# andrewli77/combinatorial-rl-tasks

Measured on NVIDIA B200. Metric: env_steps_per_sec, higher is better.
Workload: dtype f32

## Files before the change

combinatorial_rl_tasks_b200/_lib.py:

```python
import ctypes
import os

HERE = os.path.dirname(os.path.abspath(__file__))
LIB_PATH = os.environ.get('CRL_B200_LIB') or os.path.join(HERE, 'libcrl_b200.so')

c_void_p, c_int32, c_int64, c_uint32, c_uint64, c_double = (
    ctypes.c_void_p, ctypes.c_int32, ctypes.c_int64, ctypes.c_uint32, ctypes.c_uint64, ctypes.c_double)

TASK_TSP, TASK_TTSP, TASK_CM = 0, 1, 2
SEED_INCREMENT, SEED_FIXED_RANGE = 0, 1
STEP_AUTO_RESET, STEP_PHYSICS_ONLY, STEP_CHAINED, STEP_CHAIN_START, STEP_TRACK_ROWS = 1, 2, 4, 8, 16
STEP_GOALS, STEP_WAIT, STEP_ACTION_COUNTER, STEP_NO_ZONE_OBS, STEP_HOST_PLANES = 32, 64, 128, 512, 1024
STEP_ZONE_OBS_DELTA = 2048
ABI_VERSION = 9
NUM_PLANES = 23

SYMBOLS = ['crl_abi_version', 'crl_strerror', 'crl_plane_bytes', 'crl_step_bytes', 'crl_reset',
           'crl_prefetch_layouts', 'crl_prefetch_publish', 'crl_reset_from_layout', 'crl_step', 'crl_step_host',
           'crl_host_call_create', 'crl_host_call_step', 'crl_host_call_destroy',
           'crl_set_goal', 'crl_goal_query', 'crl_set_qpos_qvel',
           'crl_get_qpos_qvel', 'crl_gae', 'crl_check_state', 'crl_counters_read',
           'crl_encoder_packed_bytes', 'crl_encoder_pack', 'crl_zone_encode', 'crl_zone_encode_state',
           'crl_encoder_head_packed_bytes', 'crl_encoder_pack_head', 'crl_encoder_head',
           'crl_encoder_workspace_bytes', 'crl_encoder_forward',
           'crl_encoder_precise_packed_bytes', 'crl_encoder_pack_precise', 'crl_zone_encode_precise',
           'crl_encoder_backward_workspace_bytes', 'crl_zone_encode_backward',
           'crl_frame_capture', 'crl_zone_encode_frames', 'crl_zone_encode_backward_frames', 'crl_frames_zone_obs']
FRAME_NO_LAYOUT = 0xffffffff


class CrlConfig(ctypes.Structure):
    _fields_ = [('task', c_int32), ('num_envs', c_int32), ('num_zones', c_int32), ('num_steps', c_int32),
                ('frameskip', c_int32), ('max_cooldown', c_int32), ('seed_mode', c_int32),
# ... 36 lines not shown
            '(nvcc, sm_100a).  This package has no CPU fallback.')
    lib = ctypes.CDLL(LIB_PATH)
    P = ctypes.POINTER
    lib.crl_abi_version.restype = ctypes.c_int
    lib.crl_strerror.restype = ctypes.c_char_p
    lib.crl_strerror.argtypes = [ctypes.c_int]
    lib.crl_plane_bytes.argtypes = [P(CrlConfig), P(c_int64), c_int32]
    lib.crl_step_bytes.argtypes = [P(CrlConfig), P(c_int64), P(c_int64)]
    lib.crl_reset.argtypes = [P(CrlConfig), P(CrlState), P(CrlOut), c_void_p, c_void_p]
    lib.crl_prefetch_layouts.argtypes = [P(CrlConfig), P(CrlState), c_int32, c_uint32, c_void_p]
    lib.crl_prefetch_publish.argtypes = [P(CrlState), c_uint32, c_void_p]
    lib.crl_reset_from_layout.argtypes = [P(CrlConfig), P(CrlState), P(CrlOut), P(CrlLayoutIn), c_void_p,
                                          c_int32, c_void_p]
    lib.crl_step.argtypes = [P(CrlConfig), P(CrlState), c_void_p, P(CrlOut), c_uint32, c_uint64, c_uint64,
                             c_void_p]
    lib.crl_step_host.argtypes = [P(CrlConfig), P(CrlState), c_void_p, c_void_p, P(CrlOut), P(CrlOut),
                                  c_uint32, c_void_p]
    lib.crl_host_call_create.argtypes = [P(CrlConfig), P(CrlState), P(CrlOut), P(CrlOut), c_uint32, P(c_void_p)]
    lib.crl_host_call_step.argtypes = [c_void_p, c_void_p, c_void_p]
    lib.crl_host_call_destroy.argtypes = [c_void_p]
    lib.crl_host_call_destroy.restype = None
    lib.crl_set_goal.argtypes = [P(CrlConfig), P(CrlState), c_void_p, c_void_p]
    lib.crl_goal_query.argtypes = [P(CrlConfig), P(CrlState), c_void_p, c_void_p, c_void_p, c_void_p]
    lib.crl_set_qpos_qvel.argtypes = [P(CrlConfig), P(CrlState), c_void_p, c_void_p, c_void_p, c_int32,
                                      c_void_p]
    lib.crl_get_qpos_qvel.argtypes = [P(CrlConfig), P(CrlState), c_void_p, c_void_p, c_void_p, c_int32,
                                      c_void_p]
    lib.crl_gae.argtypes = [c_void_p, c_void_p, c_void_p, c_void_p, c_double, c_double, c_int32, c_int32,
                            c_void_p, c_void_p, c_void_p]
    lib.crl_check_state.argtypes = [P(CrlConfig), P(CrlState), c_void_p, c_void_p]
# ... 35 lines not shown
```

combinatorial_rl_tasks_b200/csrc/crl_core.cuh:

```cuda
#pragma once
#include <math.h>
#include <stdint.h>

#if defined(__CUDACC__)
#define CRL_HD __host__ __device__ __forceinline__
#define CRL_HD_COLD inline __host__ __device__ __noinline__
#else
#define CRL_HD inline
#define CRL_HD_COLD inline
#endif

namespace crl {

constexpr double kPi = 3.14159265358979323846;
constexpr double kH = 0.002;
constexpr double kMSphere = 4.0 / 3.0 * kPi * 0.1 * 0.1 * 0.1;
constexpr double kMBox = 8.0 * 0.05 * 0.05 * 0.05;
constexpr double kMass = kMSphere + kMBox;
constexpr double kCom = kMBox * 0.1 / kMass;
constexpr double kIHinge = 0.4 * kMSphere * 0.01 + kMBox / 3.0 * (0.0025 + 0.0025) + kMBox * 0.01;
constexpr double kDampLin = 0.01;
constexpr double kDampYaw = 0.005;
constexpr double kGear = 0.3;
constexpr double kForceLimit = 0.05;
// ... 207 lines not shown
#if defined(__CUDA_ARCH__)
  const double d2 = __dadd_rn(__dmul_rn(dx, dx), __dmul_rn(dy, dy));
#else
  volatile double xx = dx * dx;
  volatile double yy = dy * dy;
  const double d2 = xx + yy;
#endif
  return d2 <= thresh2;
}

CRL_HD bool near_zone(float X, float Y, float zx, float zy, float r2_guard) {
  const float dx = zx - X, dy = zy - Y;
  return dx * dx + dy * dy <= r2_guard;
}

CRL_HD int popcount32(uint32_t x) {
#if defined(__CUDA_ARCH__)
  return __popc(x);
#else
  return __builtin_popcount(x);
#endif
}

CRL_HD int hamming(uint32_t colours, int n) {
  const uint32_t field = n >= 16 ? 0x55555555u : ((1u << (2 * n)) - 1u) & 0x55555555u;
  const uint32_t lo = colours & field, hi = (colours >> 1) & field;
  const int ng = popcount32(lo & ~hi), nr = popcount32(hi & ~lo);
  const int nb = popcount32(field & ~(lo | hi));
  const int to_b = 2 * ng + nr, to_g = 2 * nr + nb, to_r = 2 * nb + ng;
  int m = to_b < to_g ? to_b : to_g;
// ... 44 lines not shown
```

combinatorial_rl_tasks_b200/csrc/crl_kernels.cu:

```cuda
#include <cuda_runtime.h>

#include <atomic>
#include <stdint.h>
#include <stdio.h>
#include <string.h>

#include "../../include/crl_b200.h"
#include "crl_core.cuh"

namespace crl {

#ifndef CRL_THREADS
#define CRL_THREADS 64
#endif
constexpr int kThreads = CRL_THREADS;
constexpr unsigned kFull = 0xffffffffu;

struct KParams {
  int B, num_steps, frameskip, max_cd, seed_mode, env_offset;
  long long min_seed, max_seed;
  double thresh2;
  float r2_guard;
  double bonus_per_step;
  double beta_a, beta_b;
// ... 23 lines not shown
  float* zone_obs_host;
  unsigned long long* result_dev;
  int32_t* goal;
  const float2* bank_zone_xy;
  const float4* bank_origin;
  const uint32_t* bank_task;
  const float4* fixed;
  uint32_t init_hi;
  uint32_t walled;
  const float2* actions;
  float4* obs;
  float* zone_obs;
  unsigned long long* result;
  float* shaped;
  const uint8_t* mask;
};

constexpr uint32_t kParBit = 0x8000u, kHiMask = 0x7fffu;

template <int TASK>
struct ZoneDim { static constexpr int Z = (TASK == CRL_TASK_TSP) ? 6 : 7; };

#ifndef CRL_REGS_N15
#define CRL_REGS_N15 112
#endif
template <int N>
struct MaxRegs { static constexpr int v = N > 8 ? CRL_REGS_N15 : 80; };

template <int N>
struct Env {
// ... 157 lines not shown

constexpr uint32_t kSlotEmpty = 0u, kSlotLayoutDone = 2u, kSlotClaimed = 3u, kSlotReady = 16u;

__device__ __forceinline__ uint32_t ld_acquire_u32(const uint32_t* p) {
  uint32_t v;
  asm volatile("ld.acquire.gpu.global.u32 %0, [%1];" : "=r"(v) : "l"(p) : "memory");
  return v;
}
__device__ __forceinline__ uint32_t ld_relaxed_u32(const uint32_t* p) {
  uint32_t v;
  asm volatile("ld.relaxed.gpu.global.u32 %0, [%1];" : "=r"(v) : "l"(p) : "memory");
  return v;
}
__device__ __forceinline__ void st_release_u32(uint32_t* p, uint32_t v) {
  asm volatile("st.release.gpu.global.u32 [%0], %1;" :: "l"(p), "r"(v) : "memory");
}

template <int TASK, int N>
__device__ __forceinline__ bool reset_from_slot(const KParams& p, int e, Env<N>& env) {
  const int B = p.B;
  const uint32_t par = env.hi >> 15;
  uint32_t episode, col_word = 0u;
  long long chosen;
  float4 o;
  uint32_t* slot_flag = nullptr;
  if (p.bank_zone_xy) {
    episode = p.episode[e];
    chosen = choose_seed(p, e, episode);
    if (chosen < p.min_seed || chosen > p.max_seed) return false;
    const size_t k = (size_t)(chosen - p.min_seed);
// ... 496 lines not shown
    row[0] = row0;
    row[1] = row1;
  }
  asm volatile("fence.proxy.async.shared::cta;" ::: "memory");
  __syncwarp();
  const int n_valid = max(0, min(32, B - warp_env0));
  if (lane == 0 && n_valid > 0) {
    const uint32_t saddr = (uint32_t)__cvta_generic_to_shared(stage);
    float4* gdst = obs + 2 * (size_t)warp_env0;
    asm volatile("cp.async.bulk.global.shared::cta.bulk_group [%0], [%1], %2;"
                 :: "l"(gdst), "r"(saddr), "r"((uint32_t)n_valid * 32u) : "memory");
    asm volatile("cp.async.bulk.commit_group;" ::: "memory");
  }
}

template <int TASK, int N>
__device__ __forceinline__ void load_env(const KParams& p, int e, Env<N>& env) {
  const float4 ps = p.pose[e];
  const float4 ax = p.aux[e];
#pragma unroll
  for (int i = 0; i < N; ++i) env.zone[i] = p.zone_xy[(size_t)i * p.B + e];
  if (TASK == CRL_TASK_TTSP) {
#pragma unroll
    for (int j = 0; j < (N + 1) / 2; ++j) env.tmax[j] = p.zone_tmax[(size_t)j * p.B + e];
  }
  if (TASK == CRL_TASK_CM) env.cd = p.cooldown[e];
  env.b.X = ps.x; env.b.Y = ps.y; env.b.phi = ps.z; env.b.vx = ps.w;
  env.b.vy = ax.x; env.b.w = ax.y; env.ep_return = ax.z;
  const uint32_t bits = (uint32_t)__float_as_int(ax.w);
  env.steps = (int)(bits & 0xffffu);
  env.hi = bits >> 16;
}

__device__ __forceinline__ double dist_np(float X, float Y, float zx, float zy) {
  const double dx = (double)zx - (double)X, dy = (double)zy - (double)Y;
  return __dsqrt_rn(__dadd_rn(__dmul_rn(dx, dx), __dmul_rn(dy, dy)));
// ... 13 lines not shown
      __nanosleep(64);
      if (++polls > (1u << 22)) { atomicAdd(p.counters + 7, 1.0); break; }
    }
  }
  __syncwarp();
}

__device__ __forceinline__ void chain_release(const KParams& p, int w, int lane, uint32_t ticket) {
  __syncwarp();
  if (lane == 0) {
    asm volatile("cp.async.bulk.wait_group 0;" ::: "memory");
    if (w < (p.B + 31) / 32) st_release_u32(p.stamp + (p.B + 31) / 32 + w, ticket + 1u);
  }
}

template <int TASK, int N, bool EXT, bool FIXED = false>
__global__ void __maxnreg__(MaxRegs<N>::v) step_kernel(const __grid_constant__ KParams p) {
  constexpr int ROW = N * ZoneDim<TASK>::Z;
  extern __shared__ __align__(128) float smem[];
  const int lane = threadIdx.x & 31, warp = threadIdx.x >> 5;
  const int e = blockIdx.x * kThreads + threadIdx.x;
  const int warp_env0 = blockIdx.x * kThreads + warp * 32;
  const bool valid = e < p.B;
  float* stage = smem + warp * (32 * ROW);
  uint32_t ticket = 0u;
  const bool ticketed = (p.flags & (CRL_STEP_CHAINED | CRL_STEP_CHAIN_START)) != 0u;
  if (ticketed) {
    ticket = chain_ticket(p, warp_env0 >> 5, lane);
    asm volatile("griddepcontrol.launch_dependents;" :: "r"(ticket) : "memory");
  } else {
    asm volatile("griddepcontrol.launch_dependents;" ::: "memory");
  }
  if (p.flags & CRL_STEP_CHAINED) {
    chain_wait(p, warp_env0 >> 5, lane, ticket);
  } else {
    asm volatile("griddepcontrol.wait;" ::: "memory");
  }

  uint32_t act_base = 0u;
  uint32_t* act_cnt = nullptr;
  if (!p.actions && (p.flags & CRL_STEP_ACTION_COUNTER) && lane == 0 && warp_env0 < p.B) {
    act_cnt = p.act_count + (warp_env0 >> 5);
    act_base = ld_relaxed_u32(act_cnt);
  }
  Env<N> env;
  float2 act = make_float2(0.f, 0.f);
  if (valid) load_env<TASK, N>(p, e, env);
  if (!p.actions && (p.flags & CRL_STEP_ACTION_COUNTER)) {
    if (act_cnt) *act_cnt = act_base + 1u;
    act_base = __shfl_sync(kFull, act_base, 0);
  }
  if (valid) {
    if (p.actions) {
      act = p.actions[e];
    } else {
      const unsigned ge = (unsigned)(p.env_offset + e);
      const unsigned long long si = p.step_index + act_base;
      U4 ctr{ge, (uint32_t)si, (uint32_t)(si >> 32), kTagAction};
      const U4 r = philox4x32(ctr, (uint32_t)p.action_seed, (uint32_t)(p.action_seed >> 32));
      act = make_float2(2.f * u01(r.x) - 1.f, 2.f * u01(r.y) - 1.f);
    }
  } else {
    env.b = Body{0.f, 0.f, 0.f, 0.f, 0.f, 0.f};
    env.ep_return = 0.f; env.steps = 0; env.hi = 0u; env.cd = make_uint2(0u, 0u);
#pragma unroll
    for (int i = 0; i < N; ++i) env.zone[i] = make_float2(1e9f, 1e9f);
#pragma unroll
    for (int j = 0; j < (N + 1) / 2; ++j) env.tmax[j] = 0xffffffffu;
  }

  const bool parked = EXT && (p.flags & CRL_STEP_WAIT) && valid && env.steps == kParkedSteps;
  const bool live = valid && !parked;
  const bool revive = EXT && parked && (p.flags & CRL_STEP_AUTO_RESET);
  const bool goals = EXT && (p.flags & CRL_STEP_GOALS);
  int goal_zone = -1;
  float gzx = 0.f, gzy = 0.f;
  double dist_before = 0.0;
  Body old_b = env.b;
  bool reached = false, park_now = false;
  if (goals && live) {
    goal_zone = p.goal[e];
// ... 3 lines not shown
      dist_before = dist_np(env.b.X, env.b.Y, gzx, gzy);
    }
  }
  int fired_out = -1;
  __shared__ unsigned s_rows_mask[kThreads / 32];
  const bool some_rows = p.zone_obs_host || (p.flags & CRL_STEP_ZONE_OBS_DELTA);
  if (some_rows && lane == 0) s_rows_mask[warp] = 0u;
  bool fresh = false;
  if (!(p.flags & CRL_STEP_PHYSICS_ONLY)) {
    bool row_changed = TASK == CRL_TASK_TTSP && !(p.flags & CRL_STEP_HOST_PLANES);
    if (TASK == CRL_TASK_CM) {
      row_changed = (env.cd.x | env.cd.y) != 0u;
      env.cd.x = cd_dec4(env.cd.x); env.cd.y = cd_dec4(env.cd.y);
    }
    uint32_t cand = 0u;
#pragma unroll
    for (int i = 0; i < N; ++i)
      if (near_zone(env.b.X, env.b.Y, env.zone[i].x, env.zone[i].y, p.r2_guard)) cand |= 1u << i;
    if (TASK == CRL_TASK_CM) {
      if (cand) {
#pragma unroll
        for (int i = 0; i < N; ++i) if (cd_get(env.cd, i) != 0u) cand &= ~(1u << i);
      }
    } else {
      cand &= ~env.hi;
    }
    int fired = -1;
    while (cand) {
      const int i = __ffs(cand) - 1;
      cand &= cand - 1u;
      float zx = 0.f, zy = 0.f;
#pragma unroll
      for (int j = 0; j < N; ++j) if (j == i) { zx = env.zone[j].x; zy = env.zone[j].y; }
      if (inside_zone(env.b.X, env.b.Y, zx, zy, p.thresh2)) { fired = i; break; }
    }
    int event = 0;
    if (fired >= 0) {
      if (TASK == CRL_TASK_CM) {
        const int old_dist = hamming(env.hi, N);
        const uint32_t col = (env.hi >> (2 * fired)) & 3u;
        const uint32_t nxt = col == 2u ? 0u : col + 1u;
        env.hi = (env.hi & ~(3u << (2 * fired))) | (nxt << (2 * fired));
        cd_set(env.cd, fired, (uint32_t)p.max_cd);
        event = old_dist - hamming(env.hi, N);
      } else {
        env.hi |= 1u << fired;
        event = 1;
      }
// ... 83 lines not shown
        if (left) {
          Env<N> next = env;
          warp_reset<TASK, N, FIXED>(p, left, lane, e, reinterpret_cast<float2*>(stage), par_in, next);
          env = next;
        }
      }
    }
  }
  float c, s;
  if (!EXT) {
    unsigned rows = 0u;
    if (some_rows) {
      __syncwarp();
      rows = s_rows_mask[warp];
    }
    if (!(p.flags & CRL_STEP_NO_ZONE_OBS) && zone_obs_step<TASK, N>(p, env, stage, lane, warp_env0, rows) && !p.zone_obs_host)
      rows = 0u;
    if (rows || p.zone_obs_host) {
      __syncwarp();
      send_rows<TASK, N>(p, p.zone_obs_host ? p.zone_obs_host : p.zone_obs, stage, rows, lane, warp_env0);
    }
    if (fresh) {
      sincosf(env.b.phi, &s, &c);
    } else {
      substeps(env.b, act.x, act.y, p.frameskip, c, s);
      env.b.phi = wrap_pi(env.b.phi);
    }
    if (p.zone_obs_host) {
      store_state_obs_host<TASK, N>(p, env, valid, e, c, s, stage, lane, warp_env0);
    } else if (valid) {
      store_state_obs<TASK, N>(p, env, e, c, s);
    }
  } else {
    if (!(p.flags & CRL_STEP_NO_ZONE_OBS))
      zone_obs_send<TASK, N>(p, env, live || revive, stage, lane, warp_env0, parked && !revive);
    if (p.zone_obs_host) send_rows<TASK, N>(p, p.zone_obs_host, stage, s_rows_mask[warp], lane, warp_env0);
    Body pb = fresh ? old_b : env.b;
    if (p.walled) substeps<CRL_CONTACT_MODEL, true>(pb, act.x, act.y, p.frameskip, c, s, p.extent);
    else substeps(pb, act.x, act.y, p.frameskip, c, s);
    if (fresh) {
      sincosf(env.b.phi, &s, &c);
    } else {
      env.b = pb;
      env.b.phi = wrap_pi(env.b.phi);
    }
    if (goals && live) {
      double shaped = 0.0;
      if (goal_zone >= 0 && !reached) {
// ... 3 lines not shown
      p.shaped[e] = (float)shaped;
    }
    if (parked && goals) p.shaped[e] = 0.f;
    if (parked && !revive) {
      p.obs[2 * (size_t)e] = make_float4(0.f, 0.f, 0.f, 0.f);
      p.obs[2 * (size_t)e + 1] = make_float4(0.f, 0.f, 0.f, 0.f);
    } else if (valid) {
      store_state_obs<TASK, N>(p, env, e, c, s, park_now);
    }
  }
  if (ticketed) {
    chain_release(p, warp_env0 >> 5, lane, ticket);
  } else {
    zone_obs_wait(lane);
  }
}

template <int TASK, int N>
__global__ void __launch_bounds__(kThreads) reset_kernel(const __grid_constant__ KParams p) {
  constexpr int ROW = N * ZoneDim<TASK>::Z;
  extern __shared__ __align__(128) float smem[];
  const int lane = threadIdx.x & 31, warp = threadIdx.x >> 5;
  const int e = blockIdx.x * kThreads + threadIdx.x;
  const int warp_env0 = blockIdx.x * kThreads + warp * 32;
  const bool valid = e < p.B;
  float* stage = smem + warp * (32 * ROW);
  Env<N> env;
  if (valid) load_env<TASK, N>(p, e, env);
  const bool want = valid && (p.mask == nullptr || p.mask[e] != 0);
  const unsigned m = __ballot_sync(kFull, want);
// ... 291 lines not shown

static int fill_params(const CrlConfig* c, const CrlState* st, const CrlOut* out, KParams& p) {
  int rc = check_config(c);
  if (rc) return rc;
  if (!st || !st->pose || !st->aux || !st->zone_xy || !st->seed || !st->episode || !st->origin || !st->counters)
    return CRL_ERR_NULL;
  if (c->task == CRL_TASK_TTSP && !st->zone_tmax) return CRL_ERR_NULL;
  if (c->task == CRL_TASK_CM && !st->cooldown) return CRL_ERR_NULL;
  if (!aligned16(st->pose) || !aligned16(st->aux) || !aligned16(st->zone_xy) || !aligned16(st->origin))
    return CRL_ERR_ALIGN;
  memset(&p, 0, sizeof(p));
  p.B = c->num_envs; p.num_steps = c->num_steps; p.frameskip = c->frameskip; p.max_cd = c->max_cooldown;
  p.seed_mode = c->seed_mode; p.env_offset = c->env_offset; p.min_seed = c->min_seed; p.max_seed = c->max_seed;
  p.thresh2 = sqrt_threshold(c->zone_size);
  p.r2_guard = (float)(c->zone_size * c->zone_size * 1.001 + 1e-5);
  p.bonus_per_step = c->time_saved_reward;
  p.beta_a = c->beta_a; p.beta_b = c->beta_b;
  p.div_steps = cached_div_const(c->num_steps, -65535, 65535);
  p.div_cd = cached_div_const(c->max_cooldown > 0 ? c->max_cooldown : 1, 0, 255);
  if (!p.div_steps.exact || !p.div_cd.exact) return CRL_ERR_CONFIG;
  p.robot_keepout = (float)c->robot_keepout; p.zone_keepout = (float)c->zone_keepout; p.extent = (float)c->extent;
  p.pose = reinterpret_cast<float4*>(st->pose); p.aux = reinterpret_cast<float4*>(st->aux);
  p.zone_xy = reinterpret_cast<float2*>(st->zone_xy); p.zone_tmax = st->zone_tmax;
  p.cooldown = reinterpret_cast<uint2*>(st->cooldown);
  p.seed = reinterpret_cast<long long*>(st->seed); p.episode = st->episode;
  p.origin = reinterpret_cast<float4*>(st->origin); p.counters = st->counters;
  if (st->next_ready) {
    if (!st->next_zone_xy || !st->next_origin || !st->next_seed || (c->task != CRL_TASK_TSP && !st->next_task))
      return CRL_ERR_NULL;
    if (!aligned16(st->next_origin) || !aligned16(st->next_zone_xy)) return CRL_ERR_ALIGN;
// ... 32 lines not shown
}

static int launch_status() { return cudaGetLastError() == cudaSuccess ? CRL_OK : CRL_ERR_LAUNCH; }

#define CRL_DISPATCH(task, n, CALL)                                              \
  do {                                                                           \
    if ((task) == CRL_TASK_TSP && (n) == 15) { CALL(CRL_TASK_TSP, 15); }         \
    else if ((task) == CRL_TASK_TSP && (n) == 5) { CALL(CRL_TASK_TSP, 5); }      \
    else if ((task) == CRL_TASK_TTSP && (n) == 15) { CALL(CRL_TASK_TTSP, 15); }  \
    else if ((task) == CRL_TASK_TTSP && (n) == 5) { CALL(CRL_TASK_TTSP, 5); }    \
    else if ((task) == CRL_TASK_CM && (n) == 6) { CALL(CRL_TASK_CM, 6); }        \
    else return CRL_ERR_UNSUPPORTED;                                             \
  } while (0)

template <int T, int NN>
static void (*pick_step_kernel(bool ext, bool fixed))(const KParams) {
  if (fixed) {
    if constexpr (T == CRL_TASK_TSP && NN == 15) return ext ? step_kernel<T, NN, true, true> : step_kernel<T, NN, false, true>;
    else return nullptr;
  }
  return ext ? step_kernel<T, NN, true> : step_kernel<T, NN, false>;
}

static int set_smem(void (*kernel)(const KParams), size_t bytes) {
  static void (*done_for[32])(const KParams) = {nullptr};
  if (bytes <= 48 * 1024) return CRL_OK;
  for (int i = 0; i < 32; ++i) {
    if (done_for[i] == kernel) return CRL_OK;
    if (done_for[i] == nullptr) {
      if (cudaFuncSetAttribute(kernel, cudaFuncAttributeMaxDynamicSharedMemorySize, (int)bytes) != cudaSuccess)
        return CRL_ERR_DEVICE;
// ... 34 lines not shown
  const int64_t B = c->num_envs, N = c->num_zones, Z = zone_dim(c->task);
  o[0] = 16 * B; o[1] = 16 * B; o[2] = 8 * N * B;
  o[3] = c->task == CRL_TASK_TTSP ? 4 * ((N + 1) / 2) * B : 0;
  o[4] = c->task == CRL_TASK_CM ? 8 * B : 0;
  o[5] = 8 * B; o[6] = 4 * B; o[7] = 16 * B; o[8] = 8 * 8;
  o[9] = 2 * 8 * N * B;
  o[10] = 2 * (c->task == CRL_TASK_TTSP ? 4 * ((N + 1) / 2) * B : (c->task == CRL_TASK_CM ? 4 * B : 0));
  o[11] = 2 * 16 * B; o[12] = 2 * 8 * B; o[13] = 2 * 4 * B;
  o[14] = 32 * B; o[15] = 4 * N * Z * B; o[16] = 8 * B;
  o[17] = 3 * 4 * ((B + 31) / 32);
  o[18] = 16 * (1 + 2 * B);
  o[19] = 16;
  o[20] = 4 * B;
  o[21] = 4 * B;
  o[22] = 16;
  for (int i = 0; i < n && i < CRL_NUM_PLANES; ++i) out_bytes[i] = o[i];
  return CRL_OK;
}

int crl_step_bytes(const CrlConfig* c, int64_t* rd, int64_t* wr) {
  int rc = check_config(c);
  if (rc) return rc;
  if (!rd || !wr) return CRL_ERR_NULL;
  const int64_t N = c->num_zones, Z = zone_dim(c->task);
  int64_t r = 8  + 32  + 8 * N, w = 32 + 8  + 32  + 4 * N * Z;
  if (c->task == CRL_TASK_TTSP) r += 4 * ((N + 1) / 2);
  if (c->task == CRL_TASK_CM) { r += 8; w += 8; }
  *rd = r; *wr = w;
  return CRL_OK;
}

static int step_launch(const CrlConfig* c, const CrlState* st, const float* actions, const CrlOut* out,
                       uint32_t flags, uint64_t action_seed, uint64_t step_index, float* zone_obs_host, void* stream,
                       CrlResult* result_dev = nullptr) {
  KParams p;
  if (!out) return CRL_ERR_NULL;
  int rc = fill_params(c, st, out, p);
  if (rc) return rc;
  p.zone_obs_host = zone_obs_host;
  p.result_dev = reinterpret_cast<unsigned long long*>(result_dev);
  if (result_dev && (!zone_obs_host || !p.row_list)) return CRL_ERR_CONFIG;
  if (actions && (reinterpret_cast<uintptr_t>(actions) & 7u)) return CRL_ERR_ALIGN;
  p.actions = reinterpret_cast<const float2*>(actions);
  p.flags = flags; p.action_seed = action_seed; p.step_index = step_index;
  const bool ticketed = (flags & (CRL_STEP_CHAINED | CRL_STEP_CHAIN_START)) != 0u;
  if (ticketed && !p.stamp) return CRL_ERR_NULL;
  if ((flags & CRL_STEP_TRACK_ROWS) && !p.row_list) return CRL_ERR_NULL;
  if ((flags & CRL_STEP_GOALS) && (!p.goal || !p.shaped)) return CRL_ERR_NULL;
  if ((flags & CRL_STEP_ACTION_COUNTER) && !p.act_count) return CRL_ERR_NULL;
  if (!(flags & CRL_STEP_NO_ZONE_OBS) && !p.zone_obs) return CRL_ERR_NULL;
  if ((flags & CRL_STEP_NO_ZONE_OBS) && (zone_obs_host || (flags & CRL_STEP_TRACK_ROWS))) return CRL_ERR_CONFIG;
  if ((flags & CRL_STEP_HOST_PLANES) && (!zone_obs_host || c->task != CRL_TASK_TTSP)) return CRL_ERR_CONFIG;
  const bool ext = (flags & (CRL_STEP_GOALS | CRL_STEP_WAIT)) != 0u || c->walled != 0u;
  if ((flags & CRL_STEP_ZONE_OBS_DELTA) && (ext || zone_obs_host || (flags & CRL_STEP_NO_ZONE_OBS))) return CRL_ERR_CONFIG;
  if (c->task == CRL_TASK_TTSP) p.flags &= ~CRL_STEP_ZONE_OBS_DELTA;
  static std::atomic<void*> last_chained_stream{reinterpret_cast<void*>(-1)};
  const bool after_chained = last_chained_stream.load(std::memory_order_relaxed) == stream;
  const bool programmatic = (flags & CRL_STEP_CHAINED) || !after_chained;
  last_chained_stream.store((flags & CRL_STEP_CHAINED) ? stream : reinterpret_cast<void*>(-1), std::memory_order_relaxed);
  const int blocks = (p.B + kThreads - 1) / kThreads;
  cudaStream_t s = static_cast<cudaStream_t>(stream);
#define CRL_CALL_STEP(T, NN)                                                        \
  {                                                                                 \
    const size_t sm = (size_t)kThreads * NN * ZoneDim<T>::Z * 4;                    \
    void (*kern)(const KParams) = pick_step_kernel<T, NN>(ext, p.fixed != nullptr); \
    if (!kern) return CRL_ERR_UNSUPPORTED;                                          \
    rc = set_smem(kern, sm);                                                        \
    if (rc) return rc;                                                              \
    cudaLaunchConfig_t lc = {};                                                     \
    lc.gridDim = dim3(blocks); lc.blockDim = dim3(kThreads);                        \
    lc.dynamicSmemBytes = sm; lc.stream = s;                                        \
    cudaLaunchAttribute at[1];                                                      \
    at[0].id = cudaLaunchAttributeProgrammaticStreamSerialization;                  \
    at[0].val.programmaticStreamSerializationAllowed = 1;                           \
    lc.attrs = at; lc.numAttrs = programmatic ? 1 : 0;                              \
    if (cudaLaunchKernelEx(&lc, kern, p) != cudaSuccess) {                          \
      (void)cudaGetLastError();                                                     \
      return CRL_ERR_LAUNCH;                                                        \
    }                                                                               \
  }
  CRL_DISPATCH(c->task, c->num_zones, CRL_CALL_STEP);
  return launch_status();
}

int crl_step(const CrlConfig* c, const CrlState* st, const float* actions, const CrlOut* out,
             uint32_t flags, uint64_t action_seed, uint64_t step_index, void* stream) {
  return step_launch(c, st, actions, out, flags, action_seed, step_index, nullptr, stream);
}

int crl_reset(const CrlConfig* c, const CrlState* st, const CrlOut* out, const uint8_t* mask, void* stream) {
  KParams p;
  if (!out || !out->zone_obs) return CRL_ERR_NULL;
  int rc = fill_params(c, st, out, p);
  if (rc) return rc;
  p.mask = mask;
  const int blocks = (p.B + kThreads - 1) / kThreads;
  cudaStream_t s = static_cast<cudaStream_t>(stream);
#define CRL_CALL_RESET(T, NN)                                                       \
  {                                                                                 \
    const size_t sm = (size_t)kThreads * NN * ZoneDim<T>::Z * 4;                    \
    rc = set_smem(reset_kernel<T, NN>, sm);                                         \
    if (rc) return rc;                                                              \
// ... 259 lines not shown
```

combinatorial_rl_tasks_b200/vec_env.py:

```python
import contextlib
import ctypes

import numpy as np
import torch

from . import _lib
from .config import ENV_SPECS
from .spaces import Box, Dict


_NO_GUARD = contextlib.nullcontext()


class _EnvView:

    def __init__(self, vec, index):
        self._vec, self.index = vec, index
        self.observation_space = vec.observation_space
        self.action_space = vec.action_space

    @property
    def unwrapped(self):
        return self

# ... 39 lines not shown
        self._write_zone_obs = True
        N, Z = spec.num_zones, spec.zone_dim
        self.cfg = _lib.CrlConfig(
            task=spec.task, num_envs=B, num_zones=N, num_steps=spec.num_steps, frameskip=spec.frameskip,
            max_cooldown=spec.max_cooldown,
            seed_mode=_lib.SEED_FIXED_RANGE if seed_mode == 'fixed_range' else _lib.SEED_INCREMENT,
            env_offset=env_offset, min_seed=min_seed, max_seed=max_seed, zone_size=spec.zone_size,
            time_saved_reward=spec.time_saved_reward, beta_a=spec.beta_a, beta_b=spec.beta_b,
            robot_keepout=spec.robot_keepout, zone_keepout=spec.zone_keepout, extent=spec.extent,
            initial_visited=spec.initial_visited, walled=1 if spec.walled else 0)
        dev = self.device
        z = lambda *shape, dtype=torch.float32: torch.zeros(*shape, dtype=dtype, device=dev)
        self.pose = z(B, 4)
        self.aux = z(B, 4)
        self.zone_xy = z(N, B, 2)
        self.zone_tmax = z((N + 1) // 2, B, dtype=torch.int32) if spec.task == _lib.TASK_TTSP else None
        self.cooldown = z(B, 2, dtype=torch.int32) if spec.task == _lib.TASK_CM else None
        self.seeds = z(B, dtype=torch.int64)
        self.episode = z(B, dtype=torch.int32)
        self.origin = z(B, 4)
        self.counters_dev = z(8, dtype=torch.float64)
        self.next_zone_xy = z(2, N, B, 2)
        if spec.task == _lib.TASK_TTSP:
            self.next_task = z(2, (N + 1) // 2, B, dtype=torch.int32)
        elif spec.task == _lib.TASK_CM:
            self.next_task = z(2, B, dtype=torch.int32)
        else:
            self.next_task = None
        self.next_origin = z(2, B, 4)
        self.next_seed = z(2, B, dtype=torch.int64)
# ... 96 lines not shown
         self.need_next_goal, self.out) = binding
        self._mirror_ok = False
        self._zone_obs_ok = False
        self._chain_ok = False

    @property
    def write_zone_obs(self):
        return self._write_zone_obs

    @write_zone_obs.setter
    def write_zone_obs(self, on):
        self._write_zone_obs = bool(on)
        self._mirror_ok = False
        self._zone_obs_ok = False

    def _guard(self):
        return _NO_GUARD if torch.cuda.current_device() == self._dev_index else torch.cuda.device(self.device)

    def _stream(self):
        return ctypes.c_void_p(_raw_stream(self._dev_index))

    def _obs_dict(self):
        return {'zone_obs': self.zone_obs, 'obs': self.obs}

    def _info(self):
        info = {'goal_met': self.goal_met, 'cost': self._cost, 'event': self.event}
        if self.spec.goals:
            info['shaped_reward'] = self.shaped_reward
            info['need_next_goal'] = self.need_next_goal
        return info
# ... 74 lines not shown
                n = xy0.shape[0]
                rot0 = self._as_dev(layout['rot0'], torch.float64).reshape(n)
                zxy = self._as_dev(layout['zone_xy'], torch.float64).reshape(n, self.spec.num_zones, 2)
                tm = self._as_dev(layout['zone_max_steps'], torch.int32) if 'zone_max_steps' in layout else None
                col = self._as_dev(layout['colours'], torch.int32) if 'colours' in layout else None
                ids = None if env_ids is None else self._as_dev(env_ids, torch.int32)
                lay = _lib.CrlLayoutIn(xy0=xy0.data_ptr(), rot0=rot0.data_ptr(), zone_xy=zxy.data_ptr(),
                                       zone_max_steps=None if tm is None else tm.data_ptr(),
                                       colours=None if col is None else col.data_ptr())
                _lib.check(self.lib.crl_reset_from_layout(self.cfg, self.state, self.out, lay,
                                                          None if ids is None else ids.data_ptr(), n,
                                                          self._stream()))
            self.gpu_launches += 1
            self._chain_ok = False
            self._mirror_ok = False
            self._zone_obs_ok = layout is None and mask is None
            if self.prefetch_every and not torch.cuda.is_current_stream_capturing():
                self.prefetch(torch.cuda.current_stream(self.device))
        return self._obs_dict()

    def _step(self, actions, flags, action_seed=0, chained=False):
        if chained:
            flags |= _lib.STEP_CHAINED if self._chain_ok else _lib.STEP_CHAIN_START
        if not flags & _lib.STEP_PHYSICS_ONLY:
            flags |= self._mode_flags
        if not self._write_zone_obs:
            flags |= _lib.STEP_NO_ZONE_OBS
        elif self._zone_obs_ok and not flags & (_lib.STEP_GOALS | _lib.STEP_WAIT) and not self.spec.walled:
            flags |= _lib.STEP_ZONE_OBS_DELTA
        with self._guard():
            if actions is None:
                aptr = None
            else:
                if not (isinstance(actions, torch.Tensor) and actions.is_cuda and actions.dtype == torch.float32
                        and actions.is_contiguous()):
                    actions = self._as_dev(actions, torch.float32)
                assert actions.shape == (self.num_envs, 2)
                aptr = actions.data_ptr()
            si = 0 if flags & _lib.STEP_ACTION_COUNTER else self._step_index
            _lib.check(self.lib.crl_step(self.cfg, self.state, aptr, self.out, flags, action_seed, si, self._stream()))
        self._step_index += 1
        self.gpu_launches += 1
        self._chain_ok = bool(chained)
        self._mirror_ok = False
        self._zone_obs_ok = self._write_zone_obs
        if self.prefetch_every and not torch.cuda.is_current_stream_capturing():
            self.tick()
        return self._obs_dict(), self.reward, self.done, self._info()

    def step(self, actions):
        return self._step(actions, (_lib.STEP_AUTO_RESET if self.auto_reset else 0) | (_lib.STEP_WAIT if self.wait else 0))

    def step_no_reset(self, actions):
        return self._step(actions, _lib.STEP_WAIT if self.wait else 0)

# ... 49 lines not shown
            pin = self._pinned.get(id(actions))
            if pin is not None:
                aptr = pin[1]
            else:
                aptr = h['actions_ptr']
                if actions is not h['np']['actions']:
                    np.copyto(h['np']['actions'], np.asarray(actions, dtype=np.float32).reshape(self.num_envs, 2))
            if torch.cuda.current_device() == self._dev_index:
                rc = self._host_call_step(call, aptr, _raw_stream(self._dev_index))
            else:
                with torch.cuda.device(self.device):
                    rc = self._host_call_step(call, aptr, _raw_stream(self._dev_index))
            if rc:
                _lib.check(rc)
            self.delta_rows = -1
            self._step_index += 1
            self.gpu_launches += 1
            self._chain_ok = False
            self._zone_obs_ok = True
            if self.prefetch_every:
                self.tick()
            return h['ret']
        hn = h['np']
        aptr = h['actions_ptr']
        if actions is not hn['actions']:
            pin = self._pinned.get(id(actions))
            if pin is not None:
                aptr = pin[1]
            else:
                np.copyto(hn['actions'], np.asarray(actions, dtype=np.float32).reshape(self.num_envs, 2))
# ... 5 lines not shown
                src = h['actions'] if aptr == h['actions_ptr'] else self._pinned[id(actions)][0]
                self._actions_dev.copy_(src, non_blocking=True)
                _lib.check(self.lib.crl_step(self.cfg, self.state, self._actions_dev.data_ptr(), self.out, flags, 0,
                                             self._step_index, self._stream()))
                h['zone_obs'].copy_(self.zone_obs.permute(2, 0, 1), non_blocking=True)
                h['obs'].copy_(self.obs, non_blocking=True)
                h['result'].copy_(self.result, non_blocking=True)
                if self.spec.goals:
                    h['shaped'].copy_(self.shaped_reward, non_blocking=True)
                torch.cuda.current_stream(self.device).synchronize()
            else:
                _lib.check(self.lib.crl_step_host(self.cfg, self.state, aptr,
                                                  self._actions_dev.data_ptr(), self.out, h['out'],
                                                  flags, self._stream()))
        self.delta_rows = self.num_envs
        self._step_index += 1
        self.gpu_launches += 1
        self._chain_ok = False
        self._mirror_ok = True
        self._zone_obs_ok = True
        if self.prefetch_every:
            self.tick()
        return h['ret']

    def _host_call(self, auto_reset, wait):
        h = self._host
        flags = (_lib.STEP_AUTO_RESET if auto_reset else 0) | (_lib.STEP_WAIT if wait else 0) | self._mode_flags
        if self.spec.task == _lib.TASK_TTSP:
            flags |= _lib.STEP_HOST_PLANES
        call = ctypes.c_void_p()
# ... 100 lines not shown
    def load_state_dict(self, d):
        assert d['env_id'] == self.env_id and d['num_envs'] == self.num_envs
        torch.cuda.current_stream(self.device).wait_stream(self._side)
        for k in self._STATE_KEYS:
            if getattr(self, k) is not None:
                getattr(self, k).copy_(d[k])
        self.cfg.num_steps = d['num_steps']
        self._step_index = d['step_index']
        self.next_ready.zero_()
        self.stamp[:2].zero_()
        if 'action_count' in d:
            self.stamp[2].copy_(d['action_count'])
        self._chain_ok = False
        self._mirror_ok = False
        self._zone_obs_ok = False
        if self.prefetch_every and self.state.bank_zone_xy is None:
            self.prefetch(torch.cuda.current_stream(self.device))

    def set_qpos_qvel(self, qpos, qvel, env_ids=None):
        qp, qv = self._as_dev(qpos, torch.float64).reshape(-1, 3), self._as_dev(qvel, torch.float64).reshape(-1, 3)
        ids = None if env_ids is None else self._as_dev(env_ids, torch.int32)
        with self._guard():
            _lib.check(self.lib.crl_set_qpos_qvel(self.cfg, self.state, qp.data_ptr(), qv.data_ptr(),
                                                  None if ids is None else ids.data_ptr(), qp.shape[0],
                                                  self._stream()))
        self._chain_ok = False
        self._mirror_ok = False
        self._zone_obs_ok = False

    def get_qpos_qvel(self, env_ids=None):
# ... 22 lines not shown
```

include/crl_b200.h:

```cpp
#ifndef CRL_B200_H_
#define CRL_B200_H_

#include <stdint.h>

#ifdef __cplusplus
extern "C" {
#endif

#define CRL_ABI_VERSION 9
#define CRL_MAX_ZONES 16

enum CrlTask { CRL_TASK_TSP = 0, CRL_TASK_TTSP = 1, CRL_TASK_CM = 2 };

enum CrlError {
  CRL_OK = 0,
  CRL_ERR_NULL = -1,
  CRL_ERR_CONFIG = -2,
  CRL_ERR_ALIGN = -3,
  CRL_ERR_UNSUPPORTED = -4,
  CRL_ERR_LAUNCH = -5,
  CRL_ERR_DEVICE = -6
};

#define CRL_STEP_AUTO_RESET 1u
// ... 75 lines not shown
  CrlResult* result;
  float* shaped_reward;
} CrlOut;

typedef struct CrlLayoutIn {
  const double* xy0;
  const double* rot0;
  const double* zone_xy;
  const int32_t* zone_max_steps;
  const int32_t* colours;
} CrlLayoutIn;

int crl_abi_version(void);
const char* crl_strerror(int code);

#define CRL_NUM_PLANES 23
int crl_plane_bytes(const CrlConfig* cfg, int64_t* out_bytes, int32_t n);

int crl_step_bytes(const CrlConfig* cfg, int64_t* bytes_read, int64_t* bytes_written);

int crl_reset(const CrlConfig* cfg, const CrlState* st, const CrlOut* out,
              const uint8_t* mask, void* stream);

int crl_prefetch_layouts(const CrlConfig* cfg, const CrlState* st, int32_t warps_per_sm,
                         uint32_t round, void* stream);
int crl_prefetch_publish(const CrlState* st, uint32_t round, void* stream);

int crl_reset_from_layout(const CrlConfig* cfg, const CrlState* st, const CrlOut* out,
                          const CrlLayoutIn* layout, const int32_t* env_ids, int32_t n,
                          void* stream);

int crl_step(const CrlConfig* cfg, const CrlState* st, const float* actions,
             const CrlOut* out, uint32_t flags, uint64_t action_seed,
             uint64_t step_index, void* stream);

int crl_step_host(const CrlConfig* cfg, const CrlState* st, const float* actions_host,
                  float* actions_dev, const CrlOut* out, const CrlOut* host_out,
                  uint32_t flags, void* stream);

typedef struct CrlHostCall CrlHostCall;
int crl_host_call_create(const CrlConfig* cfg, const CrlState* st, const CrlOut* out, const CrlOut* host_out,
                         uint32_t flags, CrlHostCall** call);
int crl_host_call_step(CrlHostCall* call, const float* actions_host, void* stream);
void crl_host_call_destroy(CrlHostCall* call);

int crl_set_goal(const CrlConfig* cfg, const CrlState* st, const int32_t* goals, void* stream);
int crl_goal_query(const CrlConfig* cfg, const CrlState* st, float* goal_xy, uint8_t* needs_goal,
                   uint8_t* available, void* stream);

// ... 73 lines not shown
```

Before: 19.42 billion.

## Screen zone proximity with packed half-precision coordinate plane in PointTSP step

Adds a persistent half2-packed copy of zone coordinates. The screened PointTSP step kernel loads this plane instead of the full float2 zone array and runs a conservative fp16 distance pre-test with a widened guard radius. Full float zone coordinates are fetched only for candidate zones and for rows that need zone observations. The goal is to cut per-step memory traffic and register use, at the cost of an extra sync kernel, a new state plane, and a dependency on the guard bound being conservative enough to keep exact hits.

```diff
diff --git a/combinatorial_rl_tasks_b200/_lib.py b/combinatorial_rl_tasks_b200/_lib.py
--- a/combinatorial_rl_tasks_b200/_lib.py
+++ b/combinatorial_rl_tasks_b200/_lib.py
@@ -13,10 +13,11 @@
 STEP_GOALS, STEP_WAIT, STEP_ACTION_COUNTER, STEP_NO_ZONE_OBS, STEP_HOST_PLANES = 32, 64, 128, 512, 1024
 STEP_ZONE_OBS_DELTA = 2048
 ABI_VERSION = 9
-NUM_PLANES = 23
+NUM_PLANES = 24
 
 SYMBOLS = ['crl_abi_version', 'crl_strerror', 'crl_plane_bytes', 'crl_step_bytes', 'crl_reset',
-           'crl_prefetch_layouts', 'crl_prefetch_publish', 'crl_reset_from_layout', 'crl_step', 'crl_step_host',
+           'crl_prefetch_layouts', 'crl_prefetch_publish', 'crl_reset_from_layout', 'crl_step', 'crl_step_screened',
+           'crl_zone_screen_sync', 'crl_step_host',
            'crl_host_call_create', 'crl_host_call_step', 'crl_host_call_destroy',
            'crl_set_goal', 'crl_goal_query', 'crl_set_qpos_qvel',
            'crl_get_qpos_qvel', 'crl_gae', 'crl_check_state', 'crl_counters_read',
@@ -83,6 +84,9 @@
                                           c_int32, c_void_p]
     lib.crl_step.argtypes = [P(CrlConfig), P(CrlState), c_void_p, P(CrlOut), c_uint32, c_uint64, c_uint64,
                              c_void_p]
+    lib.crl_step_screened.argtypes = [P(CrlConfig), P(CrlState), c_void_p, c_void_p, P(CrlOut), c_uint32, c_uint64,
+                                      c_uint64, c_void_p]
+    lib.crl_zone_screen_sync.argtypes = [P(CrlConfig), P(CrlState), c_void_p, c_void_p]
     lib.crl_step_host.argtypes = [P(CrlConfig), P(CrlState), c_void_p, c_void_p, P(CrlOut), P(CrlOut),
                                   c_uint32, c_void_p]
     lib.crl_host_call_create.argtypes = [P(CrlConfig), P(CrlState), P(CrlOut), P(CrlOut), c_uint32, P(c_void_p)]
diff --git a/combinatorial_rl_tasks_b200/csrc/crl_core.cuh b/combinatorial_rl_tasks_b200/csrc/crl_core.cuh
--- a/combinatorial_rl_tasks_b200/csrc/crl_core.cuh
+++ b/combinatorial_rl_tasks_b200/csrc/crl_core.cuh
@@ -1,6 +1,10 @@
 #pragma once
 #include <math.h>
 #include <stdint.h>
+#include <string.h>
+#if defined(__CUDACC__)
+#include <cuda_fp16.h>
+#endif
 
 #if defined(__CUDACC__)
 #define CRL_HD __host__ __device__ __forceinline__
@@ -245,6 +249,90 @@
   return dx * dx + dy * dy <= r2_guard;
 }
 
+constexpr uint16_t kHalfNaN = 0x7e00u;
+
+inline double half_rn_host(double v) {
+  if (v != v) return v;
+  const double a = fabs(v);
+  if (a >= 65520.0) return copysign(INFINITY, v);
+  int ex;
+  frexp(a, &ex);
+  const double ulp = ldexp(1.0, (ex - 1 > -14 ? ex - 1 : -14) - 10);
+  return copysign(nearbyint(a / ulp) * ulp, v);
+}
+
+inline uint16_t half_bits_host(double h) {
+  if (h != h) return kHalfNaN;
+  const uint16_t s = signbit(h) ? 0x8000u : 0u;
+  const double a = fabs(h);
+  if (a == INFINITY) return s | 0x7c00u;
+  if (a < ldexp(1.0, -14)) return s | (uint16_t)(a * ldexp(1.0, 24));
+  int ex;
+  const double m = frexp(a, &ex);
+  return s | (uint16_t)((ex + 14) << 10) | (uint16_t)((m * 2.0 - 1.0) * 1024.0);
+}
+
+inline double half_value_host(uint16_t b) {
+  const int e = (b >> 10) & 0x1f, m = b & 0x3ff;
+  const double s = (b & 0x8000u) ? -1.0 : 1.0;
+  if (e == 0x1f) return m ? NAN : s * INFINITY;
+  if (e == 0) return s * ldexp((double)m, -24);
+  return s * ldexp(1024.0 + m, e - 25);
+}
+
+CRL_HD uint16_t screen_coord(float z) {
+  if (!(fabsf(z) < 4.f)) return kHalfNaN;
+#if defined(__CUDA_ARCH__)
+  return __half_as_ushort(__float2half_rn(z));
+#else
+  return half_bits_host(half_rn_host((double)z));
+#endif
+}
+
+CRL_HD void screen_pair(float xa, float ya, float xb, float yb, uint32_t& wx, uint32_t& wy) {
+  wx = (uint32_t)screen_coord(xa) | ((uint32_t)screen_coord(xb) << 16);
+  wy = (uint32_t)screen_coord(ya) | ((uint32_t)screen_coord(yb) << 16);
+}
+
+CRL_HD uint32_t screen_robot(float v) {
+#if defined(__CUDA_ARCH__)
+  const __half2 h = __float2half2_rn(v);
+  return *reinterpret_cast<const uint32_t*>(&h);
+#else
+  const uint32_t b = half_bits_host(half_rn_host((double)v));
+  return b | (b << 16);
+#endif
+}
+
+CRL_HD uint32_t screen_pair_pass(uint32_t wx, uint32_t wy, uint32_t X2, uint32_t Y2, uint32_t g2) {
+#if defined(__CUDA_ARCH__)
+  const __half2 dx = __hsub2(*reinterpret_cast<const __half2*>(&wx), *reinterpret_cast<const __half2*>(&X2));
+  const __half2 dy = __hsub2(*reinterpret_cast<const __half2*>(&wy), *reinterpret_cast<const __half2*>(&Y2));
+  const __half2 d2 = __hfma2(dx, dx, __hmul2(dy, dy));
+  const uint32_t m = __hleu2_mask(d2, *reinterpret_cast<const __half2*>(&g2));
+  return (m & 1u) | ((m >> 15) & 2u);
+#else
+  uint32_t out = 0u;
+  for (int k = 0; k < 2; ++k) {
+    const int sh = 16 * k;
+    const double dx = half_rn_host(half_value_host((uint16_t)(wx >> sh)) - half_value_host((uint16_t)(X2 >> sh)));
+    const double dy = half_rn_host(half_value_host((uint16_t)(wy >> sh)) - half_value_host((uint16_t)(Y2 >> sh)));
+    const double d2 = half_rn_host(dx * dx + half_rn_host(dy * dy));
+    if (!(d2 > half_value_host((uint16_t)(g2 >> sh)))) out |= 1u << k;
+  }
+  return out;
+#endif
+}
+
+inline uint32_t screen_g2(double r) {
+  const double rr = r * (1.0 + ldexp(1.0, -51)) + 3.0 * 1.4142135623730951 * ldexp(1.0, -10);
+  const double g = rr * rr * (1.0 + ldexp(1.0, -8));
+  double h = half_rn_host(g);
+  if (h < g) h = half_value_host((uint16_t)(half_bits_host(h) + 1u));
+  const uint32_t b = half_bits_host(h);
+  return b | (b << 16);
+}
+
 CRL_HD int popcount32(uint32_t x) {
 #if defined(__CUDA_ARCH__)
   return __popc(x);
diff --git a/combinatorial_rl_tasks_b200/csrc/crl_kernels.cu b/combinatorial_rl_tasks_b200/csrc/crl_kernels.cu
--- a/combinatorial_rl_tasks_b200/csrc/crl_kernels.cu
+++ b/combinatorial_rl_tasks_b200/csrc/crl_kernels.cu
@@ -61,6 +61,8 @@
   unsigned long long* result;
   float* shaped;
   const uint8_t* mask;
+  uint2* zone_screen;
+  uint32_t screen_g2;
 };
 
 constexpr uint32_t kParBit = 0x8000u, kHiMask = 0x7fffu;
@@ -248,6 +250,16 @@
 }
 __device__ __forceinline__ void st_release_u32(uint32_t* p, uint32_t v) {
   asm volatile("st.release.gpu.global.u32 [%0], %1;" :: "l"(p), "r"(v) : "memory");
+}
+
+template <int N>
+__device__ __forceinline__ void store_screen(const KParams& p, int e, const float2* z) {
+#pragma unroll
+  for (int j = 0; j < (N + 1) / 2; ++j) {
+    uint2 w;
+    screen_pair(z[2 * j].x, z[2 * j].y, 2 * j + 1 < N ? z[2 * j + 1].x : 0.f, 2 * j + 1 < N ? z[2 * j + 1].y : 0.f, w.x, w.y);
+    p.zone_screen[(size_t)j * p.B + e] = w;
+  }
 }
 
 template <int TASK, int N>
@@ -774,12 +786,17 @@
   }
 }
 
-template <int TASK, int N>
-__device__ __forceinline__ void load_env(const KParams& p, int e, Env<N>& env) {
+template <int TASK, int N, bool SCREEN = false>
+__device__ __forceinline__ void load_env(const KParams& p, int e, Env<N>& env, uint2* scr = nullptr) {
   const float4 ps = p.pose[e];
   const float4 ax = p.aux[e];
-#pragma unroll
-  for (int i = 0; i < N; ++i) env.zone[i] = p.zone_xy[(size_t)i * p.B + e];
+  if (SCREEN) {
+#pragma unroll
+    for (int j = 0; j < (N + 1) / 2; ++j) scr[j] = p.zone_screen[(size_t)j * p.B + e];
+  } else {
+#pragma unroll
+    for (int i = 0; i < N; ++i) env.zone[i] = p.zone_xy[(size_t)i * p.B + e];
+  }
   if (TASK == CRL_TASK_TTSP) {
 #pragma unroll
     for (int j = 0; j < (N + 1) / 2; ++j) env.tmax[j] = p.zone_tmax[(size_t)j * p.B + e];
@@ -823,8 +840,9 @@
   }
 }
 
-template <int TASK, int N, bool EXT, bool FIXED = false>
+template <int TASK, int N, bool EXT, bool FIXED = false, bool SCREEN = false>
 __global__ void __maxnreg__(MaxRegs<N>::v) step_kernel(const __grid_constant__ KParams p) {
+  static_assert(!(SCREEN && (EXT || TASK != CRL_TASK_TSP)), "the screened step is the plain PointTSP kernel");
   constexpr int ROW = N * ZoneDim<TASK>::Z;
   extern __shared__ __align__(128) float smem[];
   const int lane = threadIdx.x & 31, warp = threadIdx.x >> 5;
@@ -853,8 +871,9 @@
     act_base = ld_relaxed_u32(act_cnt);
   }
   Env<N> env;
+  uint2 scr[(N + 1) / 2];
   float2 act = make_float2(0.f, 0.f);
-  if (valid) load_env<TASK, N>(p, e, env);
+  if (valid) load_env<TASK, N, SCREEN>(p, e, env, scr);
   if (!p.actions && (p.flags & CRL_STEP_ACTION_COUNTER)) {
     if (act_cnt) *act_cnt = act_base + 1u;
     act_base = __shfl_sync(kFull, act_base, 0);
@@ -874,6 +893,8 @@
     env.ep_return = 0.f; env.steps = 0; env.hi = 0u; env.cd = make_uint2(0u, 0u);
 #pragma unroll
     for (int i = 0; i < N; ++i) env.zone[i] = make_float2(1e9f, 1e9f);
+#pragma unroll
+    for (int j = 0; j < (N + 1) / 2; ++j) scr[j] = make_uint2(0x7bff7bffu, 0x7bff7bffu);
 #pragma unroll
     for (int j = 0; j < (N + 1) / 2; ++j) env.tmax[j] = 0xffffffffu;
   }
@@ -907,9 +928,16 @@
       env.cd.x = cd_dec4(env.cd.x); env.cd.y = cd_dec4(env.cd.y);
     }
     uint32_t cand = 0u;
-#pragma unroll
-    for (int i = 0; i < N; ++i)
-      if (near_zone(env.b.X, env.b.Y, env.zone[i].x, env.zone[i].y, p.r2_guard)) cand |= 1u << i;
+    if (SCREEN) {
+      const uint32_t X2 = screen_robot(env.b.X), Y2 = screen_robot(env.b.Y);
+#pragma unroll
+      for (int j = 0; j < (N + 1) / 2; ++j) cand |= screen_pair_pass(scr[j].x, scr[j].y, X2, Y2, p.screen_g2) << (2 * j);
+      cand &= (1u << N) - 1u;
+    } else {
+#pragma unroll
+      for (int i = 0; i < N; ++i)
+        if (near_zone(env.b.X, env.b.Y, env.zone[i].x, env.zone[i].y, p.r2_guard)) cand |= 1u << i;
+    }
     if (TASK == CRL_TASK_CM) {
       if (cand) {
 #pragma unroll
@@ -923,8 +951,13 @@
       const int i = __ffs(cand) - 1;
       cand &= cand - 1u;
       float zx = 0.f, zy = 0.f;
-#pragma unroll
-      for (int j = 0; j < N; ++j) if (j == i) { zx = env.zone[j].x; zy = env.zone[j].y; }
+      if (SCREEN) {
+        const float2 z = p.zone_xy[(size_t)i * p.B + e];
+        zx = z.x; zy = z.y;
+      } else {
+#pragma unroll
+        for (int j = 0; j < N; ++j) if (j == i) { zx = env.zone[j].x; zy = env.zone[j].y; }
+      }
       if (inside_zone(env.b.X, env.b.Y, zx, zy, p.thresh2)) { fired = i; break; }
     }
     int event = 0;
@@ -1038,6 +1071,11 @@
       __syncwarp();
       rows = s_rows_mask[warp];
     }
+    if (SCREEN && ((rows >> lane) & 1u)) {
+#pragma unroll
+      for (int i = 0; i < N; ++i) env.zone[i] = p.zone_xy[(size_t)i * p.B + e];
+    }
+    if (TASK == CRL_TASK_TSP && p.zone_screen && fresh) store_screen<N>(p, e, env.zone);
     if (!(p.flags & CRL_STEP_NO_ZONE_OBS) && zone_obs_step<TASK, N>(p, env, stage, lane, warp_env0, rows) && !p.zone_obs_host)
       rows = 0u;
     if (rows || p.zone_obs_host) {
@@ -1056,6 +1094,7 @@
       store_state_obs<TASK, N>(p, env, e, c, s);
     }
   } else {
+    if (TASK == CRL_TASK_TSP && p.zone_screen && fresh) store_screen<N>(p, e, env.zone);
     if (!(p.flags & CRL_STEP_NO_ZONE_OBS))
       zone_obs_send<TASK, N>(p, env, live || revive, stage, lane, warp_env0, parked && !revive);
     if (p.zone_obs_host) send_rows<TASK, N>(p, p.zone_obs_host, stage, s_rows_mask[warp], lane, warp_env0);
@@ -1089,6 +1128,16 @@
   } else {
     zone_obs_wait(lane);
   }
+}
+
+template <int N>
+__global__ void __launch_bounds__(128) zone_screen_sync_kernel(const KParams p) {
+  const int e = blockIdx.x * blockDim.x + threadIdx.x;
+  if (e >= p.B) return;
+  float2 z[N];
+#pragma unroll
+  for (int i = 0; i < N; ++i) z[i] = p.zone_xy[(size_t)i * p.B + e];
+  store_screen<N>(p, e, z);
 }
 
 template <int TASK, int N>
@@ -1410,6 +1459,7 @@
   p.seed_mode = c->seed_mode; p.env_offset = c->env_offset; p.min_seed = c->min_seed; p.max_seed = c->max_seed;
   p.thresh2 = sqrt_threshold(c->zone_size);
   p.r2_guard = (float)(c->zone_size * c->zone_size * 1.001 + 1e-5);
+  p.screen_g2 = screen_g2(c->zone_size);
   p.bonus_per_step = c->time_saved_reward;
   p.beta_a = c->beta_a; p.beta_b = c->beta_b;
   p.div_steps = cached_div_const(c->num_steps, -65535, 65535);
@@ -1472,7 +1522,14 @@
   } while (0)
 
 template <int T, int NN>
-static void (*pick_step_kernel(bool ext, bool fixed))(const KParams) {
+static void (*pick_step_kernel(bool ext, bool fixed, bool screen))(const KParams) {
+  if constexpr (T == CRL_TASK_TSP) {
+    if (screen && !ext) {
+      if (!fixed) return step_kernel<T, NN, false, false, true>;
+      if constexpr (NN == 15) return step_kernel<T, NN, false, true, true>;
+      else return nullptr;
+    }
+  }
   if (fixed) {
     if constexpr (T == CRL_TASK_TSP && NN == 15) return ext ? step_kernel<T, NN, true, true> : step_kernel<T, NN, false, true>;
     else return nullptr;
@@ -1537,6 +1594,7 @@
   o[20] = 4 * B;
   o[21] = 4 * B;
   o[22] = 16;
+  o[23] = c->task == CRL_TASK_TSP ? 8 * ((N + 1) / 2) * B : 0;
   for (int i = 0; i < n && i < CRL_NUM_PLANES; ++i) out_bytes[i] = o[i];
   return CRL_OK;
 }
@@ -1555,11 +1613,13 @@
 
 static int step_launch(const CrlConfig* c, const CrlState* st, const float* actions, const CrlOut* out,
                        uint32_t flags, uint64_t action_seed, uint64_t step_index, float* zone_obs_host, void* stream,
-                       CrlResult* result_dev = nullptr) {
+                       CrlResult* result_dev = nullptr, uint32_t* zone_screen = nullptr) {
   KParams p;
   if (!out) return CRL_ERR_NULL;
   int rc = fill_params(c, st, out, p);
   if (rc) return rc;
+  if (zone_screen && (reinterpret_cast<uintptr_t>(zone_screen) & 7u)) return CRL_ERR_ALIGN;
+  if (c->task == CRL_TASK_TSP) p.zone_screen = reinterpret_cast<uint2*>(zone_screen);
   p.zone_obs_host = zone_obs_host;
   p.result_dev = reinterpret_cast<unsigned long long*>(result_dev);
   if (result_dev && (!zone_obs_host || !p.row_list)) return CRL_ERR_CONFIG;
@@ -1577,6 +1637,7 @@
   const bool ext = (flags & (CRL_STEP_GOALS | CRL_STEP_WAIT)) != 0u || c->walled != 0u;
   if ((flags & CRL_STEP_ZONE_OBS_DELTA) && (ext || zone_obs_host || (flags & CRL_STEP_NO_ZONE_OBS))) return CRL_ERR_CONFIG;
   if (c->task == CRL_TASK_TTSP) p.flags &= ~CRL_STEP_ZONE_OBS_DELTA;
+  const bool screen = p.zone_screen && (p.flags & CRL_STEP_ZONE_OBS_DELTA);
   static std::atomic<void*> last_chained_stream{reinterpret_cast<void*>(-1)};
   const bool after_chained = last_chained_stream.load(std::memory_order_relaxed) == stream;
   const bool programmatic = (flags & CRL_STEP_CHAINED) || !after_chained;
@@ -1586,7 +1647,7 @@
 #define CRL_CALL_STEP(T, NN)                                                        \
   {                                                                                 \
     const size_t sm = (size_t)kThreads * NN * ZoneDim<T>::Z * 4;                    \
-    void (*kern)(const KParams) = pick_step_kernel<T, NN>(ext, p.fixed != nullptr); \
+    void (*kern)(const KParams) = pick_step_kernel<T, NN>(ext, p.fixed != nullptr, screen); \
     if (!kern) return CRL_ERR_UNSUPPORTED;                                          \
     rc = set_smem(kern, sm);                                                        \
     if (rc) return rc;                                                              \
@@ -1609,6 +1670,27 @@
 int crl_step(const CrlConfig* c, const CrlState* st, const float* actions, const CrlOut* out,
              uint32_t flags, uint64_t action_seed, uint64_t step_index, void* stream) {
   return step_launch(c, st, actions, out, flags, action_seed, step_index, nullptr, stream);
+}
+
+int crl_step_screened(const CrlConfig* c, const CrlState* st, uint32_t* zone_screen, const float* actions,
+                      const CrlOut* out, uint32_t flags, uint64_t action_seed, uint64_t step_index, void* stream) {
+  if (!zone_screen && c && c->task == CRL_TASK_TSP) return CRL_ERR_NULL;
+  return step_launch(c, st, actions, out, flags, action_seed, step_index, nullptr, stream, nullptr, zone_screen);
+}
+
+int crl_zone_screen_sync(const CrlConfig* c, const CrlState* st, uint32_t* zone_screen, void* stream) {
+  KParams p;
+  int rc = fill_params(c, st, nullptr, p);
+  if (rc) return rc;
+  if (c->task != CRL_TASK_TSP) return CRL_OK;
+  if (!zone_screen) return CRL_ERR_NULL;
+  if (reinterpret_cast<uintptr_t>(zone_screen) & 7u) return CRL_ERR_ALIGN;
+  p.zone_screen = reinterpret_cast<uint2*>(zone_screen);
+  const int blocks = (p.B + 127) / 128;
+  cudaStream_t s = static_cast<cudaStream_t>(stream);
+#define CRL_CALL_SCREEN_SYNC(T, NN) { if (T == CRL_TASK_TSP) zone_screen_sync_kernel<NN><<<blocks, 128, 0, s>>>(p); }
+  CRL_DISPATCH(c->task, c->num_zones, CRL_CALL_SCREEN_SYNC);
+  return launch_status();
 }
 
 int crl_reset(const CrlConfig* c, const CrlState* st, const CrlOut* out, const uint8_t* mask, void* stream) {
diff --git a/combinatorial_rl_tasks_b200/vec_env.py b/combinatorial_rl_tasks_b200/vec_env.py
--- a/combinatorial_rl_tasks_b200/vec_env.py
+++ b/combinatorial_rl_tasks_b200/vec_env.py
@@ -77,6 +77,8 @@
         self.pose = z(B, 4)
         self.aux = z(B, 4)
         self.zone_xy = z(N, B, 2)
+        self._zone_screen = z((N + 1) // 2, B, 2, dtype=torch.int32) if spec.task == _lib.TASK_TSP else None
+        self._screen_ok = False
         self.zone_tmax = z((N + 1) // 2, B, dtype=torch.int32) if spec.task == _lib.TASK_TTSP else None
         self.cooldown = z(B, 2, dtype=torch.int32) if spec.task == _lib.TASK_CM else None
         self.seeds = z(B, dtype=torch.int64)
@@ -203,6 +205,16 @@
         self._mirror_ok = False
         self._zone_obs_ok = False
 
+    @property
+    def _screen_ptr(self):
+        return None if self._zone_screen is None else self._zone_screen.data_ptr()
+
+    def screen_sync(self):
+        with self._guard():
+            _lib.check(self.lib.crl_zone_screen_sync(self.cfg, self.state, self._screen_ptr, self._stream()))
+        self.gpu_launches += 1
+        self._screen_ok = True
+
     def _guard(self):
         return _NO_GUARD if torch.cuda.current_device() == self._dev_index else torch.cuda.device(self.device)
 
@@ -307,6 +319,7 @@
             self.gpu_launches += 1
             self._chain_ok = False
             self._mirror_ok = False
+            self._screen_ok = False
             self._zone_obs_ok = layout is None and mask is None
             if self.prefetch_every and not torch.cuda.is_current_stream_capturing():
                 self.prefetch(torch.cuda.current_stream(self.device))
@@ -330,8 +343,11 @@
                     actions = self._as_dev(actions, torch.float32)
                 assert actions.shape == (self.num_envs, 2)
                 aptr = actions.data_ptr()
+            if flags & _lib.STEP_ZONE_OBS_DELTA and not self._screen_ok:
+                self.screen_sync()
             si = 0 if flags & _lib.STEP_ACTION_COUNTER else self._step_index
-            _lib.check(self.lib.crl_step(self.cfg, self.state, aptr, self.out, flags, action_seed, si, self._stream()))
+            _lib.check(self.lib.crl_step_screened(self.cfg, self.state, self._screen_ptr, aptr, self.out, flags,
+                                                  action_seed, si, self._stream()))
         self._step_index += 1
         self.gpu_launches += 1
         self._chain_ok = bool(chained)
@@ -411,6 +427,7 @@
             if rc:
                 _lib.check(rc)
             self.delta_rows = -1
+            self._screen_ok = False
             self._step_index += 1
             self.gpu_launches += 1
             self._chain_ok = False
@@ -446,6 +463,7 @@
                                                   self._actions_dev.data_ptr(), self.out, h['out'],
                                                   flags, self._stream()))
         self.delta_rows = self.num_envs
+        self._screen_ok = False
         self._step_index += 1
         self.gpu_launches += 1
         self._chain_ok = False
@@ -576,6 +594,7 @@
         self._chain_ok = False
         self._mirror_ok = False
         self._zone_obs_ok = False
+        self._screen_ok = False
         if self.prefetch_every and self.state.bank_zone_xy is None:
             self.prefetch(torch.cuda.current_stream(self.device))
 
diff --git a/include/crl_b200.h b/include/crl_b200.h
--- a/include/crl_b200.h
+++ b/include/crl_b200.h
@@ -113,7 +113,7 @@
 int crl_abi_version(void);
 const char* crl_strerror(int code);
 
-#define CRL_NUM_PLANES 23
+#define CRL_NUM_PLANES 24
 int crl_plane_bytes(const CrlConfig* cfg, int64_t* out_bytes, int32_t n);
 
 int crl_step_bytes(const CrlConfig* cfg, int64_t* bytes_read, int64_t* bytes_written);
@@ -132,6 +132,12 @@
 int crl_step(const CrlConfig* cfg, const CrlState* st, const float* actions,
              const CrlOut* out, uint32_t flags, uint64_t action_seed,
              uint64_t step_index, void* stream);
+
+int crl_step_screened(const CrlConfig* cfg, const CrlState* st, uint32_t* zone_screen,
+                      const float* actions, const CrlOut* out, uint32_t flags,
+                      uint64_t action_seed, uint64_t step_index, void* stream);
+
+int crl_zone_screen_sync(const CrlConfig* cfg, const CrlState* st, uint32_t* zone_screen, void* stream);
 
 int crl_step_host(const CrlConfig* cfg, const CrlState* st, const float* actions_host,
                   float* actions_dev, const CrlOut* out, const CrlOut* host_out,
```

Result: faster. 20.08 billion, median of 6 (+3.4%).
